# Shamir-Lab/Faucet

Measured on AMD Instinct MI355X. Metric: canonical k-mers/s (load+scan) at k=31, 100bp reads; % HBM roofline, higher is better.
Workload: dtype u64

## Files before the change

### faucet_amd/csrc/api.hip

```cpp
#include <cstdio>
#include <algorithm>
#include <string>

#include <chrono>
#include <thread>

#include "fgpu_ctx.h"

int fgpu_scan_export_impl(fgpu_ctx* ctx, void* dev_entries, uint64_t cap_entries, uint64_t* d_stamps, uint64_t* n_entries);
int fgpu_scan_import_impl(fgpu_ctx* ctx, const void* dev_entries, uint64_t n);
int fgpu_scan_download_impl(fgpu_ctx* ctx, uint64_t* keys_host, fgpu_junction* recs_host, uint64_t cap, uint64_t* n_out);

static thread_local std::string g_create_error;

int g_fgpu_trace = getenv("FGPU_TRACE") && getenv("FGPU_TRACE")[0] == '1';

int fgpu_ensure(fgpu_ctx* ctx, DevBuf* b, uint64_t bytes) {
    if (b->bytes >= bytes && b->p) return FGPU_OK;
    if (b->p) {
        FGPU_HIP(fgpu_sync_stream(ctx, ctx->stream));
        FGPU_HIP(hipFree(b->p));
        b->p = nullptr;
        b->bytes = 0;
    } else {
// ... 568 lines not shown
    ctx->host_waits = 0;
    ctx->host_wait_ms = 0;
    ctx->wait_sites.clear();
    if (ctx->short_pf) FGPU_HIP(hipMemsetAsync(ctx->short_pf, 0, ctx->short_pf_tai / 8, ctx->stream));
    if ((rc = fgpu_long_pairs_reset(ctx))) return rc;
    ctx->have_import = false;
    ctx->journal_max_read_len = 0;
    ctx->hint_in_table = false;
    ctx->hint_gen = 0;
    ctx->hint_n = ctx->hint_max_seq = 0;
    ctx->delta_ready = false;
    ctx->delta_keys = ctx->refresh_full = ctx->refresh_delta = ctx->refresh_mismatch = 0;
    ctx->sparse_links = ctx->full_links = 0;
    ctx->dbg_stall_us = getenv("FGPU_DEBUG_WALK_STALL_US") ? std::min(100000, std::max(0, atoi(getenv("FGPU_DEBUG_WALK_STALL_US")))) : 0;
    ctx->dbg_delta_check = getenv("FGPU_DEBUG_DELTA_CHECK") != nullptr;
    ctx->no_sparse_link = getenv("FGPU_NO_SPARSE_LINK") != nullptr;
    const uint64_t start_span = std::max<uint64_t>(1ULL << 18, ctx->settled_span / 4);
    ctx->window_span = ctx->prm.walk_window_span ? std::min<uint64_t>(std::max<uint64_t>(ctx->prm.walk_window_span, 64), ctx->max_span)
                                                 : std::min<uint64_t>(start_span, ctx->max_span);
    ctx->calib_left = 16;
    ctx->calib_f = ctx->calib_p = 0;
    ctx->adapt_followers = 0;
    ctx->adapt_pieces = 0;
    ctx->adapt_overflows = 0;
    ctx->adapt_vote = 0;
    ctx->calib_ovf = 0;
    ctx->span_ceiling = ~0ULL;
    ctx->repeats_seen_before = false;
    ctx->walked_pieces = 0;
    ctx->scan_batch_index = 0;
// ... 109 lines not shown
        int rc = pull_counters(ctx);
        if (rc) return rc;
        BatchBufs* const cur = ctx->cur;
        ctx->journal_max_read_len = std::max<uint64_t>(ctx->journal_max_read_len, ctx->counters_host->max_read_len);
        if (ctx->lazy_failed && (rc = scan_replay(ctx))) return rc;
        ctx->cur = cur;
        ctx->journal_on = false;
        ctx->eager_scan = true;
        journal_recycle(ctx);
        return FGPU_OK;
    }
    JournalBatch* j;
    if (!ctx->journal_pool.empty()) { j = ctx->journal_pool.back(); ctx->journal_pool.pop_back(); }
    else j = new JournalBatch();
    int rc;
    if ((rc = fgpu_ensure_b(ctx, &j->codes, cb)) || (rc = fgpu_ensure_b(ctx, &j->bad, bbytes)) || (ob && (rc = fgpu_ensure_b(ctx, &j->offs, ob)))) {
        ctx->journal_pool.push_back(j);
        return rc;
    }
    if (b->T) {
        FGPU_HIP(hipMemcpyAsync(j->codes.p, b->codes.p, cb, hipMemcpyDeviceToDevice, ctx->stream));
        FGPU_HIP(hipMemcpyAsync(j->bad.p, b->bad.p, bbytes, hipMemcpyDeviceToDevice, ctx->stream));
        if (ob) FGPU_HIP(hipMemcpyAsync(j->offs.p, b->d_offs, ob, hipMemcpyDeviceToDevice, ctx->stream));
    }
    j->T = b->T; j->n_words = b->n_words; j->n_reads = b->n_reads; j->seq = b->seq;
    ctx->journal.push_back(j);
    ctx->journal_bytes += cb + bbytes + ob;
    (void)reads;
    return FGPU_OK;
}

static int scan_replay_once(fgpu_ctx* ctx);
static int scan_replay(fgpu_ctx* ctx) {
    for (int attempt = 0;; attempt++) {
        const bool for_room = ctx->capacity_failed;
        ctx->capacity_failed = false;
        if (for_room) {
            int rc = sync_all(ctx);
// ... 12 lines not shown
}

static int scan_replay_once(fgpu_ctx* ctx) {
    ctx->in_replay = true;
    ctx->journal_on = false;
    ctx->eager_scan = true;
    ctx->lazy_failed = false;
    int rc = sync_all(ctx);
    for (BatchBufs* b : ctx->prepared) ctx->pool.push_back(b);
    ctx->prepared.clear();
    for (BatchBufs* b : ctx->to_harvest) b->stops_pending = false;
    ctx->to_harvest.clear();
    stop_queue_recycle(ctx);
    if (!rc) rc = fgpu_scan_reset(ctx);
    if (rc) { ctx->in_replay = false; return rc; }
    {
        unsigned long long ln[3] = {0, 0, 0};
        if (hipMemcpy(ln, ctx->counters->late_n, sizeof(ln), hipMemcpyDeviceToHost) == hipSuccess)
            for (int i = 0; i < 3; i++) ctx->late_acc[i] += ln[i];
    }
    FGPU_HIP(hipMemsetAsync(ctx->counters, 0, sizeof(DevCounters), ctx->stream));
    FGPU_HIP(hipMemcpyAsync(&ctx->counters->max_read_len, &ctx->journal_max_read_len, 8, hipMemcpyHostToDevice, ctx->stream));
    FGPU_HIP(fgpu_sync_stream(ctx, ctx->stream));
    const uint64_t reads_processed = ctx->scan_stats.reads_processed;
    memset(&ctx->scan_stats, 0, sizeof(ctx->scan_stats));
    ctx->scan_stats.reads_processed = reads_processed;
    memset(ctx->counters_host, 0, sizeof(DevCounters));
    ctx->scan_windows = 0;
    ctx->scan_pieces_seen = 0;
    ctx->scan_piece_base = 0;
// ... 28 lines not shown
        if (b->stops_pending && (rc = fgpu_scan_harvest(ctx, b))) {
            ctx->pool.push_back(b);
            break;
        }
        if (b->walk_pending) {
            FGPU_HIP(fgpu_sync_event(ctx, b->walk_done));
            b->walk_pending = false;
        }
        b->seq = j->seq;
        ctx->cur = b;
        b->T = j->T; b->n_words = j->n_words; b->n_reads = j->n_reads;
        b->d_offs = (const uint64_t*)j->offs.p;
        if (b->T) {
            const uint64_t cb = 2 * (b->n_words + FGPU_PADW) * 8, bbytes = (b->n_words + FGPU_PADW) * 8;
            if ((rc = fgpu_ensure_b(ctx, &b->codes, cb)) || (rc = fgpu_ensure_b(ctx, &b->bad, bbytes))) break;
            FGPU_HIP(hipMemcpyAsync(b->codes.p, j->codes.p, cb, hipMemcpyDeviceToDevice, ctx->stream));
            FGPU_HIP(hipMemcpyAsync(b->bad.p, j->bad.p, bbytes, hipMemcpyDeviceToDevice, ctx->stream));
        }
        uint64_t n_pieces = 0;
        rc = fgpu_stage_scan_pure(ctx, &n_pieces);
        if (!rc) rc = check_errors(ctx);
        if (!rc && b->pure_done) FGPU_HIP(hipEventRecord(b->pure_done, ctx->stream));
        if (!rc) rc = fgpu_scan_reserve(ctx, ctx->counters_host->n_junctions + ctx->scan_imported);
        if (!rc) {
            adapt_window(ctx);
            rc = fgpu_stage_scan_walk(ctx, b->n_pieces);
            ctx->walked_pieces += b->n_pieces;
            if (!rc) note_walked(ctx, b);
        }
        ctx->pool.push_back(b);
    }
    ctx->cur = &ctx->bb_default;
// ... 206 lines not shown
    if (dbg_host) {
        fprintf(stderr, "[host] scan: wait for the buffers' last walk %.2f ms, pack issue %.2f, pure stage issue (first half) %.2f, wait for the piece count %.2f, "
                        "pure stage issue (second half) %.2f, walk issue %.2f\n", ctx->host_ms[0], ctx->host_ms[1], ctx->host_ms[2], ctx->host_ms[3], ctx->host_ms[4], ctx->host_ms[5]);
        for (double& v : ctx->host_ms) v = 0;
    }
    int rc = pull_counters(ctx);
    if (!rc && ctx->lazy_failed) {
        rc = scan_replay(ctx);
        if (!rc) rc = pull_counters(ctx);
    }
    while (!rc && !ctx->to_harvest.empty()) rc = fgpu_scan_harvest(ctx, ctx->to_harvest.front());
    if (!rc) rc = fgpu_long_pairs_close(ctx);
    ctx->phase = 0;
    ctx->journal_on = false;
    if (!rc && !ctx->prm.walk_window_span && ctx->scan_windows > 8) ctx->settled_span = ctx->window_span;
    if (rc) return rc;
    const DevCounters& c = *ctx->counters_host;
    fgpu_scan_stats& s = ctx->scan_stats;
    s.unambiguous_reads = c.segments + ctx->carried.unambiguous_reads;
    s.reads_no_errors = c.pieces + ctx->carried.reads_no_errors;
    s.nb_jcheck_kmer = c.nb_jcheck + ctx->carried.nb_jcheck_kmer;
    s.nb_no_juncs = c.nb_no_juncs + ctx->carried.nb_no_juncs;
    s.nb_processed = c.nb_processed + ctx->carried.nb_processed;
    s.nb_skipped = c.nb_skipped + ctx->carried.nb_skipped;
    s.n_junctions = c.n_junctions + ctx->scan_imported;
    s.kmers = c.kmers + ctx->carried.kmers;
    s.reads_processed += ctx->carried.reads_processed;
    s.walk_windows = ctx->scan_windows;
    s.walk_followers = c.followers;
    s.walk_max_cluster = c.max_cluster;
// ... 285 lines not shown
```

### faucet_amd/csrc/fgpu_ctx.h

```cpp
#pragma once
#include <chrono>
#include <hip/hip_runtime.h>
#include <stdint.h>
#include <stdio.h>
#include <string.h>

#include <string>
#include <thread>
#include <vector>

#include "../../include/faucet_gpu.h"
#include <deque>

#include "fgpu_device.h"

#define FGPU_PADW 8
#define FGPU_USUAL_SPAN (1ULL << 26)
#define FGPU_MAX_SPAN (1ULL << 26)

struct DevBuf {
    void*    p = nullptr;
    uint64_t bytes = 0;
};

// ... 32 lines not shown

struct ResidentBatch {
    DevBuf codes, bad, sure;
    DevBuf fail;
    uint64_t T = 0, n_words = 0;
    uint32_t tb = 0;
};

struct DeltaList {
    DevBuf list, count;
};
#define FGPU_DELTA_RING 4

struct JournalBatch {
    DevBuf codes, bad, offs;
    uint64_t T = 0, n_words = 0, n_reads = 0, seq = 0;
};
#define FGPU_INTERNAL_REPLAY 1000

struct StopBatch {
    uint64_t seq = 0;
    fgpu_stop* data = nullptr;
    size_t n = 0, cap = 0;
};

struct LongPairs {
    int mode = 0;
    uint64_t tai = 0;
    int n_hash = 0;
    uint32_t* bits = nullptr;
// ... 158 lines not shown
    uint64_t scan_piece_base = 0;
    uint64_t scan_imported = 0;
    bool hint_in_table = false;
    uint32_t hint_gen = 0;
    uint64_t hint_n = 0, hint_max_seq = 0;
    uint64_t hint_digest[2] = {0, 0};
    DevBuf delta_filter;
    uint64_t delta_filter_bits = 0;
    bool delta_ready = false;
    uint64_t delta_keys = 0;
    uint64_t refresh_full = 0, refresh_delta = 0, refresh_mismatch = 0;
    DevBuf cand_filter;
    uint64_t sparse_links = 0, full_links = 0;
    int dbg_stall_us = 0;
    bool dbg_delta_check = false;
    bool no_sparse_link = false;
    DevBuf import_probe;
    uint64_t scan_grown = 0;

    DevCounters* counters = nullptr;
    DevCounters* counters_host = nullptr;

    fgpu_load_stats load_stats;
    uint64_t load_mark_hits = 0, load_mark_pending = 0;
    fgpu_scan_stats scan_stats;
    uint64_t scan_windows = 0;
    uint64_t scan_pieces_seen = 0;

    uint64_t adapt_followers = 0, adapt_pieces = 0;
    double host_ms[8] = {0, 0, 0, 0, 0, 0, 0, 0};
// ... 2 lines not shown
    uint64_t span_ceiling = ~0ULL;
    int adapt_vote = 0;
    uint64_t proven_span = 0;
    uint64_t adapt_overflows = 0;
    int calib_left = 0;
    uint64_t calib_f = 0, calib_p = 0;
    unsigned long long* fb_host = nullptr;
    fgpu_scan_stats carried = {};

    BatchBufs bb_default;
    BatchBufs* cur = &bb_default;
    std::vector<BatchBufs*> prepared;
    std::vector<BatchBufs*> pool;
    std::vector<BatchBufs*> all_batches;
    std::vector<JournalBatch*> journal, journal_pool;
    uint64_t journal_bytes = 0, journal_budget = 0;
    bool journal_on = false;
    bool eager_scan = false;
    bool lazy_failed = false;
    bool in_replay = false;
    bool capacity_failed = false;
    uint64_t capacity_replays = 0;
    uint32_t* short_pf = nullptr;
    uint64_t short_pf_tai = 0;
    int short_pf_hashes = 0;
    bool short_pf_lists_to_host = true;
    LongPairs lp;
    uint64_t stops_delivered = 0;
    uint64_t lp_applied_seq = 0;
    uint64_t scan_replays = 0;
// ... 155 lines not shown
```

### faucet_amd/csrc/load.hip

```cpp
#include <algorithm>

#include "fgpu_ctx.h"
#include "fgpu_flags.h"

namespace {

__device__ __forceinline__ void wave_add(unsigned long long* dst, unsigned long long v) {
    for (int o = 32; o > 0; o >>= 1) v += __shfl_down(v, o, 64);
    if (fd_lane() == 0 && v) atomicAdd(dst, v);
}

__device__ __forceinline__ void block_add(unsigned long long* dst, unsigned long long v) {
    __shared__ unsigned long long part[4];
    for (int o = 32; o > 0; o >>= 1) v += __shfl_down(v, o, 64);
    if (fd_lane() == 0) part[threadIdx.x >> 6] = v;
    __syncthreads();
    if (threadIdx.x == 0) {
        const unsigned long long t = part[0] + part[1] + part[2] + part[3];
        if (t) atomicAdd(dst, t);
    }
    __syncthreads();
}

#ifdef FGPU_FIRST_MASK_LOG2
// ... 561 lines not shown
    if (ctx->resident_bytes + cb + 2 * pb + (ctx->shard_planes ? MISS_PLANES * pb : 0) > ctx->resident_budget) {
        ctx->resident_open = false;
        return FGPU_OK;
    }
    if (ctx->resident_count == ctx->resident.size()) ctx->resident.push_back(new ResidentBatch());
    ResidentBatch& r = *ctx->resident[ctx->resident_count];
    const uint64_t fb = ctx->shard_planes ? MISS_PLANES * pb : 0;
    if (fgpu_ensure_b(ctx, &r.codes, cb) || fgpu_ensure_b(ctx, &r.bad, pb) || fgpu_ensure_b(ctx, &r.sure, pb) || (fb && fgpu_ensure_b(ctx, &r.fail, fb))) {
        (void)hipGetLastError();
        ctx->resident_open = false;
        return FGPU_OK;
    }
    r.T = bb.T;
    r.n_words = bb.n_words;
    r.tb = ctx->cur_tb;
    FGPU_HIP(hipMemcpyAsync(r.codes.p, bb.codes.p, cb, hipMemcpyDeviceToDevice, ctx->stream));
    FGPU_HIP(hipMemcpyAsync(r.bad.p, bb.bad.p, pb, hipMemcpyDeviceToDevice, ctx->stream));
    FGPU_HIP(hipMemcpyAsync(r.sure.p, bb.sure.p, pb, hipMemcpyDeviceToDevice, ctx->stream));
    if (fb) FGPU_HIP(hipMemcpyAsync(r.fail.p, bb.fail.p, fb, hipMemcpyDeviceToDevice, ctx->stream));
    ctx->resident_count++;
    ctx->resident_bytes += cb + 2 * pb + fb;
    return FGPU_OK;
}

int fgpu_load_sweep(fgpu_ctx* ctx) {
    if (ctx->epoch_positions == 0) return FGPU_OK;
    if (ctx->rec_layout) FGPU_LAUNCH("carry_update", k_carry_from_rec, 8192, 256, ctx->rec, ctx->prm.tai / 32);
    else FGPU_LAUNCH("carry_update", k_carry_from_first, 4096, 256, ctx->pair, (const uint4*)ctx->first, ctx->prm.tai);
    ctx->swept_positions += ctx->epoch_positions;
    ctx->epoch_positions = 0;
    return FGPU_OK;
}

int fgpu_stage_load(fgpu_ctx* ctx) {
// ... 133 lines not shown
```

### faucet_amd/csrc/scan_pure.hip

```cpp
#include <algorithm>

#include "fgpu_ctx.h"
#include "fgpu_flags.h"

namespace {

__device__ __forceinline__ void wave_add(unsigned long long* dst, unsigned long long v) {
    for (int o = 32; o > 0; o >>= 1) v += __shfl_down(v, o, 64);
    if (fd_lane() == 0 && v) atomicAdd(dst, v);
}

__device__ __forceinline__ void block_add(unsigned long long* dst, unsigned long long v) {
    __shared__ unsigned long long part[4];
    for (int o = 32; o > 0; o >>= 1) v += __shfl_down(v, o, 64);
    if (fd_lane() == 0) part[threadIdx.x >> 6] = v;
    __syncthreads();
    if (threadIdx.x == 0) {
        const unsigned long long t = part[0] + part[1] + part[2] + part[3];
        if (t) atomicAdd(dst, t);
    }
    __syncthreads();
}

__global__ void __launch_bounds__(256) k_scan_same(const uint64_t* __restrict__ codes, const uint64_t* __restrict__ kept_codes, uint64_t n_code_words,
                                                   const uint64_t* __restrict__ bad, const uint64_t* __restrict__ kept_bad, uint64_t n_words,
                                                   uint32_t* same) {
    bool differ = false;
    for (uint64_t i = (uint64_t)blockIdx.x * blockDim.x + threadIdx.x; i < n_code_words; i += (uint64_t)gridDim.x * blockDim.x) {
        differ |= codes[i] != kept_codes[i];
        if (i < n_words) differ |= bad[i] != kept_bad[i];
    }
    if (__ballot(differ) && fd_lane() == 0) *same = 0;
}

__global__ void __launch_bounds__(256) k_scan_valid(const uint64_t* __restrict__ codes, const uint64_t* __restrict__ bad,
                                                    uint64_t T, uint64_t n_words, FdParams fp, const uint32_t* __restrict__ bloom,
                                                    const uint64_t* __restrict__ sure, const uint32_t* __restrict__ same,
                                                    uint64_t* __restrict__ valid, DevCounters* cnt) {
    unsigned long long n_ok = 0, n_reused = 0;
    const uint64_t total = n_words * 64;
    const bool reuse = sure && *same != 0;
    for (uint64_t p = (uint64_t)blockIdx.x * blockDim.x + threadIdx.x; p < total; p += (uint64_t)gridDim.x * blockDim.x) {
        bool ok = p < T && fd_window_ok(bad, p, fp.k);
        bool v = false;
        if (ok) {
            n_ok++;
            if (reuse && ((sure[p >> 6] >> (p & 63)) & 1ULL)) {
// ... 427 lines not shown

}

void fgpu_touch_scan_pure() {
    hipFuncAttributes attr;
    (void)hipFuncGetAttributes(&attr, (const void*)k_scan_same);
}

int fgpu_util_probe_stage3(fgpu_ctx* ctx, const uint64_t* d_kmers, uint64_t n, int mode, signed char* d_out) {
    FGPU_LAUNCH("probe_stage3", k_probe_stage3, fgpu_blocks(n, 256), 256, d_kmers, n, mode, ctx->fd, (const uint32_t*)ctx->bloo2, d_out);
    return FGPU_OK;
}

int fgpu_stage_scan_pure(fgpu_ctx* ctx, uint64_t* n_pieces) {
    BatchBufs& bb = *ctx->cur;
    *n_pieces = 0;
    bb.n_pieces = 0;
    if (bb.T == 0) return FGPU_OK;
    const uint64_t wb = (bb.n_words + FGPU_PADW) * 8;
    int rc;
    DevBuf* planes[] = {&bb.valid, &bb.pm, &bb.ps, &bb.ff, &bb.fb, &bb.cf0, &bb.cf1, &bb.cb0, &bb.cb1, &bb.inF, &bb.inB, &bb.lk, &bb.nF, &bb.nB, &bb.need};
    for (DevBuf* b : planes)
        if ((rc = fgpu_ensure_b(ctx, b, wb))) return rc;
    if ((rc = fgpu_ensure_b(ctx, &bb.ps_prefix, (bb.n_words + FGPU_PADW + bb.n_words / SCAN_BLOCK + 2) * 4))) return rc;
    const double t_a = fgpu_host_now();
    FGPU_HIP(hipMemsetAsync(bb.valid.p, 0, wb, ctx->stream));
    FGPU_HIP(hipMemsetAsync(bb.pm.p, 0, wb, ctx->stream));
    FGPU_HIP(hipMemsetAsync(bb.ps.p, 0, wb, ctx->stream));

    const unsigned grid = fgpu_grid(bb.n_words * 64, 256);
    const unsigned wgrid = fgpu_grid(bb.n_words, 256);
    if ((rc = fgpu_util_count_segments(ctx, ctx->fd.k + 2 * ctx->fd.j + 1))) return rc;
    const ResidentBatch* kept = ctx->scan_batch_index < ctx->resident_count ? ctx->resident[ctx->scan_batch_index] : nullptr;
    ctx->scan_batch_index++;
    if (kept && (kept->T != bb.T || kept->n_words != bb.n_words)) kept = nullptr;
    if (kept) {
        if ((rc = fgpu_ensure_b(ctx, &bb.same, 64))) return rc;
        FGPU_HIP(hipMemsetAsync(bb.same.p, 0x01, 4, ctx->stream));
        const uint64_t ncw = 2 * bb.n_words;
        FGPU_LAUNCH("scan_same", k_scan_same, fgpu_grid(ncw, 256), 256, (const uint64_t*)bb.codes.p, (const uint64_t*)kept->codes.p, ncw,
                    (const uint64_t*)bb.bad.p, (const uint64_t*)kept->bad.p, bb.n_words, (uint32_t*)bb.same.p);
    }
    FGPU_LAUNCH("scan_valid", k_scan_valid, grid, 256, (const uint64_t*)bb.codes.p, (const uint64_t*)bb.bad.p, bb.T, bb.n_words, ctx->fd,
                (const uint32_t*)ctx->bloo2, kept ? (const uint64_t*)kept->sure.p : (const uint64_t*)nullptr,
                kept ? (const uint32_t*)bb.same.p : (const uint32_t*)nullptr, (uint64_t*)bb.valid.p, ctx->counters);
    const int check_segment = ctx->fd.k < 2 * ctx->fd.j + 2;
    FGPU_LAUNCH("scan_pieces", k_scan_pieces, wgrid, 256, (const uint64_t*)bb.valid.p, (const uint64_t*)bb.bad.p, bb.n_words, ctx->fd,
                check_segment, (unsigned long long*)bb.pm.p, (uint64_t*)bb.ps.p, ctx->counters);
    uint32_t* prefix = (uint32_t*)bb.ps_prefix.p;
    uint32_t* block_sums = prefix + bb.n_words + FGPU_PADW;
    const uint32_t nblk = fgpu_blocks(bb.n_words + 1, SCAN_BLOCK);
    const uint64_t nw1 = bb.n_words + 1;
    FGPU_LAUNCH("prefix_block", k_prefix_block, nblk, SCAN_BLOCK, (const uint64_t*)bb.ps.p, nw1, prefix, block_sums);
    FGPU_LAUNCH("prefix_sums", k_prefix_sums, 1, SCAN_BLOCK, block_sums, nblk);
    FGPU_LAUNCH("prefix_apply", k_prefix_apply, fgpu_blocks(nw1, 256), 256, prefix, (const uint32_t*)block_sums, nw1);
    FGPU_HIP(hipMemcpyAsync(ctx->counters_host, ctx->counters, sizeof(DevCounters), hipMemcpyDeviceToHost, ctx->stream));
// ... 48 lines not shown
```

### faucet_amd/csrc/scan_walk.hip

```cpp
#include <cstring>
#include <algorithm>

#include "fgpu_ctx.h"
#include "fgpu_flags.h"

#include <rocprim/rocprim.hpp>

namespace {

constexpr uint64_t J_EMPTY = ~0ULL;
constexpr uint64_t J_KEYMASK = (1ULL << 62) - 1;
constexpr uint32_t U_INF = 0xFFFFFFFFu;
constexpr uint64_t J_PROBE_LIMIT = 1ULL << 14;
constexpr int STAMP_SHIFT = 20;
constexpr uint64_t STAMP_FAKE = (1ULL << STAMP_SHIFT) - 1;

struct JTable {
    uint64_t* keys;
    uint8_t* recs;
    uint64_t* stamps;
    uint64_t mask;
    uint32_t* filter;
    uint64_t filter_mask;
};
// ... 83 lines not shown
    }
    return false;
}

__device__ __forceinline__ uint32_t uf_find(uint32_t* parent, uint32_t x) {
    uint32_t p = ld_agent(&parent[x]);
    while (p != x) {
        uint32_t gp = ld_agent(&parent[p]);
        if (gp != p) atomicMin(&parent[x], gp);
        x = p;
        p = gp;
    }
    return x;
}

__device__ __forceinline__ void uf_union(uint32_t* parent, uint32_t a, uint32_t b) {
    for (;;) {
        a = uf_find(parent, a);
        b = uf_find(parent, b);
        if (a == b) return;
        if (a < b) { uint32_t t = a; a = b; b = t; }
        uint32_t old = atomicCAS(&parent[a], a, b);
        if (old == a) return;
    }
}

constexpr int W_OWNER_BITS = 24;
constexpr uint64_t W_OWNER_MASK = (1ULL << W_OWNER_BITS) - 1;
constexpr uint64_t W_EPOCH_MASK = 0xFFULL << 56;
constexpr uint32_t W_NO_OWNER = (uint32_t)W_OWNER_MASK;
__device__ __forceinline__ uint32_t wt_filter_bit(const WTable& wt, uint32_t h32) { return (h32 * 0x85EBCA6Bu) >> wt.fshift; }

__device__ __forceinline__ void wt_register(const WTable& wt, uint32_t* parent, uint32_t h32, uint32_t piece, DevCounters* cnt) {
    const unsigned long long mine = (unsigned long long)(wt.epoch | ((uint64_t)h32 << W_OWNER_BITS) | (uint64_t)piece);
    uint64_t s = (uint64_t)h32 & wt.mask;
    for (uint64_t n = 0; n <= wt.mask; n++) {
        unsigned long long v = wt.keys[s];
        if ((v & W_EPOCH_MASK) != wt.epoch) {
// ... 62 lines not shown

struct DeltaSrc {
    const uint32_t* list[FGPU_DELTA_RING];
    const unsigned long long* count[FGPU_DELTA_RING];
};

__global__ void __launch_bounds__(256) k_walk_register(Planes pl, FdParams fp, WTable wt, uint32_t* parent, uint64_t lo, uint64_t hi,
                                                       uint64_t pos_end, DevCounters* cnt, unsigned word_blocks, unsigned piece_blocks, DeltaSrc ds) {
    const WinDesc wd = make_window(pl, lo, hi);
    if (blockIdx.x < word_blocks) {
        const uint64_t w = (wd.lo >> 6) + (uint64_t)blockIdx.x * blockDim.x + threadIdx.x;
        if (w * 64 >= pos_end) return;
        unsigned long long m = pl.pm[w] & (pl.inF[w] | pl.inB[w] | pl.ff[w] | pl.fb[w]);
        if (w == (wd.lo >> 6)) m &= ~0ULL << (wd.lo & 63);
        if ((w + 1) * 64 > pos_end) m &= (1ULL << (pos_end & 63)) - 1;
        while (m) {
            const int b = __builtin_ctzll(m);
            m &= m - 1;
            const uint64_t p = w * 64 + (uint64_t)b;
            uint32_t li;
            uint2 pc;
            if (piece_in_window(pl, wd, p, li, pc)) wt_register(wt, parent, pl.kh[p], li, cnt);
        }
    } else if (blockIdx.x < word_blocks + piece_blocks) {
        const uint32_t li = (blockIdx.x - word_blocks) * blockDim.x + threadIdx.x;
        if (li >= wd.n) return;
        const uint2 pc = pl.pieces[wd.first_piece + li];
        const uint32_t len = pc.y + (uint32_t)fp.k - 1;
        wt_register(wt, parent, pl.kh[pc.x + (len / 2 - (uint32_t)fp.k / 2)], li, cnt);
        for (uint32_t q = (uint32_t)fp.max_spacer - 1; q < pc.y; q++) wt_register(wt, parent, pl.kh[pc.x + q], li, cnt);
    } else {
        const uint64_t t = (uint64_t)(blockIdx.x - word_blocks - piece_blocks) * blockDim.x + threadIdx.x;
        const uint64_t stride = (uint64_t)(gridDim.x - word_blocks - piece_blocks) * blockDim.x;
        for (int r = 0; r < FGPU_DELTA_RING; r++) {
            if (!ds.list[r]) continue;
            const uint64_t n = *ds.count[r];
            for (uint64_t i = t; i < n; i += stride) wt_register(wt, nullptr, ds.list[r][i], W_NO_OWNER, cnt);
        }
    }
}

__global__ void __launch_bounds__(256) k_walk_link(Planes pl, FdParams fp, WTable wt, uint32_t* parent, uint64_t lo, uint64_t hi,
                                                   uint64_t pos_end, uint32_t* roots_state) {
    const WinDesc wd = make_window(pl, lo, hi);
    if (roots_state && blockIdx.x == 0 && threadIdx.x == 0) { roots_state[0] = 0; roots_state[1] = 0; }
    const uint64_t base0 = wd.lo & ~63ULL;
    constexpr int U = 4;
    for (uint64_t base = base0 + (uint64_t)blockIdx.x * (256 * U); base < pos_end; base += (uint64_t)gridDim.x * (256 * U)) {
        uint64_t p[U];
        uint32_t h[U], fw[U];
        bool act[U];
#pragma unroll
        for (int u = 0; u < U; u++) {
            p[u] = base + (uint64_t)u * 256 + threadIdx.x;
            act[u] = p[u] >= wd.lo && p[u] < pos_end && ((pl.pm[p[u] >> 6] >> (p[u] & 63)) & 1ULL);
        }
#pragma unroll
        for (int u = 0; u < U; u++) h[u] = act[u] ? pl.kh[p[u]] : 0u;
#pragma unroll
        for (int u = 0; u < U; u++) {
            const uint32_t b = wt_filter_bit(wt, h[u]);
            fw[u] = act[u] ? ((wt.bits[b >> 5] >> (b & 31)) & 1u) : 0u;
        }
#pragma unroll
        for (int u = 0; u < U; u++) {
            bool hit = false;
            if (fw[u]) {
                uint64_t slot = 0;
                uint32_t owner = wt_owner(wt, h[u], slot);
                if (owner != U_INF) {
                    uint32_t li;
                    uint2 pc;
                    if (piece_in_window(pl, wd, p[u], li, pc)) {
                        hit = true;
                        if (owner == W_NO_OWNER) {
                            const unsigned long long mine = (unsigned long long)(wt.epoch | ((uint64_t)h[u] << W_OWNER_BITS) | (uint64_t)li);
                            owner = (uint32_t)(atomicMin((unsigned long long*)&wt.keys[slot], mine) & W_OWNER_MASK);
                        }
                        if (owner != li && owner != W_NO_OWNER) uf_union(parent, li, owner);
                    }
                }
            }
            const uint64_t m = __ballot(hit);
            if (fd_lane() == 0 && p[u] < ((pos_end + 63) & ~63ULL)) pl.lk[p[u] >> 6] = m;
        }
    }
}

constexpr int CAND_FILTER_LOG2 = 27;
__device__ __forceinline__ uint32_t cand_bit(uint32_t h32) { return (h32 * 0xC2B2AE35u) >> (32 - CAND_FILTER_LOG2); }

__global__ void __launch_bounds__(256) k_cand_mark(const uint64_t* __restrict__ pm, const uint64_t* __restrict__ inF, const uint64_t* __restrict__ inB,
                                                   const uint64_t* __restrict__ ff, const uint64_t* __restrict__ fb, const uint32_t* __restrict__ kh,
                                                   uint64_t n_words, const uint2* __restrict__ pieces, uint64_t n_pieces, FdParams fp,
                                                   uint32_t* __restrict__ filt, unsigned word_blocks) {
    if (blockIdx.x < word_blocks) {
        for (uint64_t w = (uint64_t)blockIdx.x * blockDim.x + threadIdx.x; w < n_words; w += (uint64_t)word_blocks * blockDim.x) {
            unsigned long long m = pm[w] & (inF[w] | inB[w] | ff[w] | fb[w]);
            while (m) {
// ... 55 lines not shown
            if (!piece_in_window(pl, wd, p, li, pc)) continue;
            out |= 1ULL << b;
            if (owner == W_NO_OWNER) {
                const unsigned long long mine = (unsigned long long)(wt.epoch | ((uint64_t)h << W_OWNER_BITS) | (uint64_t)li);
                owner = (uint32_t)(atomicMin((unsigned long long*)&wt.keys[slot], mine) & W_OWNER_MASK);
            }
            if (owner != li && owner != W_NO_OWNER) uf_union(parent, li, owner);
        }
        lk_out[w] = out;
    }
}

__global__ void __launch_bounds__(256) k_walk_cluster(const uint32_t* __restrict__ parent, uint32_t* count, uint32_t* head,
                                                      uint32_t* __restrict__ flat, uint32_t* __restrict__ next, Planes pl, uint64_t lo,
                                                      uint64_t hi, WinDesc* wd_out, DevCounters* cnt, uint32_t* weight, uint32_t heavy_w,
                                                      uint32_t* __restrict__ root_list, uint32_t* roots_state) {
    const WinDesc wd = make_window(pl, lo, hi);
    const uint32_t n = wd.n;
    if (blockIdx.x == 0 && threadIdx.x == 0) {
        *wd_out = wd;
        cnt->pad2 = 0;
    }
    for (uint32_t i = blockIdx.x * blockDim.x + threadIdx.x; i < n; i += gridDim.x * blockDim.x) {
        uint32_t r = i;
        for (;;) { uint32_t pr = parent[r]; if (pr == r) break; r = pr; }
        flat[i] = r;
        if (r != i) {
            next[i] = atomicExch(&head[r], i);
            atomicAdd(&count[r], 1u);
        }
        {
            const bool is_root = r == i;
            const unsigned long long m = __ballot(is_root);
            if (m) {
                const int first = __builtin_ctzll(m);
// ... 1800 lines not shown
            const unsigned total = s_wave[0] + s_wave[1] + s_wave[2] + s_wave[3];
            s_base = total ? atomicAdd(count, (unsigned long long)total) : 0ULL;
        }
        __syncthreads();
        unsigned long long at = s_base + (incl - mine);
        for (int q = 0; q < wave; q++) at += s_wave[q];
        while (m) {
            const int b = __builtin_ctzll(m);
            m &= m - 1;
            list[at++] = kh[w * 64 + (uint64_t)b];
        }
        __syncthreads();
    }
}

__global__ void __launch_bounds__(256) k_walk_reset_uf(uint32_t* parent, uint32_t* count, uint32_t* head, uint32_t* par_fail, uint32_t n, uint4* wbits,
                                                       uint32_t wbits_vec) {
    for (uint32_t a = blockIdx.x * blockDim.x + threadIdx.x; a < n; a += gridDim.x * blockDim.x) {
        parent[a] = a;
        count[a] = 0;
        head[a] = U_INF;
        par_fail[a] = 0;
    }
    for (uint32_t a = blockIdx.x * blockDim.x + threadIdx.x; a < wbits_vec; a += gridDim.x * blockDim.x) wbits[a] = make_uint4(0, 0, 0, 0);
}

__global__ void __launch_bounds__(256) k_fill_u64(uint64_t* p, uint64_t n, uint64_t v) {
    uint64_t i = (uint64_t)blockIdx.x * blockDim.x + threadIdx.x;
    uint64_t stride = (uint64_t)gridDim.x * blockDim.x;
    for (; i < n; i += stride) p[i] = v;
}
__global__ void __launch_bounds__(256) k_iota_u32(uint32_t* p, uint64_t n) {
// ... 657 lines not shown
                    }
                if (lo) {
                    ds.list[FGPU_DELTA_RING - 1] = (const uint32_t*)mine_list.list.p;
                    ds.count[FGPU_DELTA_RING - 1] = (const unsigned long long*)mine_list.count.p;
                }
            }
            const unsigned word_blocks = fgpu_blocks((pos_end - (lo & ~63ULL) + 63) / 64, 256);
            const unsigned piece_blocks = fgpu_blocks(max_pieces, 256);
            static const unsigned delta_per_block = getenv("FGPU_DELTA_PER_BLOCK") ? (unsigned)std::max(1, atoi(getenv("FGPU_DELTA_PER_BLOCK"))) : 1024u;
            const unsigned delta_blocks = refresh_window ? 64u : (unsigned)std::min<uint64_t>(4096, std::max<uint64_t>(64, delta_est / delta_per_block));
            FGPU_LAUNCH("walk_lookup", k_walk_register, word_blocks + piece_blocks + delta_blocks, 256, pl, ctx->fd, wt, uf_parent, lo, hi, pos_end, ctx->counters,
                        word_blocks, piece_blocks, ds);
        }
        uint32_t* const roots_state = ctx->cl_roots;
        uint32_t* const root_list = ctx->cl_roots + 16;
        if (cand_ok && lo == 0) {
            const uint64_t link_words = ((pos_end + 63) >> 6) - (lo >> 6);
            FGPU_LAUNCH("walk_link", k_walk_link_sparse, std::min(fgpu_blocks(link_words, 256), 4096u), 256, pl, ctx->fd, wt, uf_parent, lo, hi, pos_end, roots_state,
                        (const uint64_t*)bb.cand.p, (uint64_t*)bb.lk.p);
            ctx->sparse_links++;
            if (ctx->dbg_delta_check) {
                uint64_t* copy = nullptr;
                unsigned long long* out = nullptr;
                FGPU_HIP(hipMalloc(&copy, link_words * 8));
                FGPU_HIP(hipMalloc(&out, 32));
                FGPU_HIP(hipMemsetAsync(out, 0, 32, walk_stream));
                FGPU_HIP(hipMemcpyAsync(copy, (const uint64_t*)bb.lk.p + (lo >> 6), link_words * 8, hipMemcpyDeviceToDevice, walk_stream));
                hipLaunchKernelGGL(k_walk_link, dim3(std::min(fgpu_blocks(pos_end - (lo & ~63ULL), 1024), 4096u)), dim3(256), 0, walk_stream, pl, ctx->fd, wt, uf_parent, lo, hi, pos_end,
                                   (uint32_t*)nullptr);
                hipLaunchKernelGGL(k_dbg_diff, dim3(64), dim3(256), 0, walk_stream, (const uint64_t*)copy, (const uint64_t*)bb.lk.p + (lo >> 6), link_words, out, 0);
                unsigned long long h[4] = {0, 0, 0, 0};
                FGPU_HIP(hipMemcpyAsync(h, out, 32, hipMemcpyDeviceToHost, walk_stream));
                FGPU_HIP(hipStreamSynchronize(walk_stream));
                ctx->refresh_mismatch += h[0];
                if (h[0]) fprintf(stderr, "[fgpu] sparse link pass: %llu lk words differ from the full pass's, batch %llu window at %llu\n", h[0], (unsigned long long)bb.seq, (unsigned long long)lo);
                (void)hipFree(copy); (void)hipFree(out);
            }
        } else {
            FGPU_LAUNCH("walk_link", k_walk_link, std::min(fgpu_blocks(pos_end - (lo & ~63ULL), 1024), 4096u), 256, pl, ctx->fd, wt, uf_parent, lo, hi, pos_end, roots_state);
            if (ctx->refresh_snapshot) ctx->full_links++;
        }
        const uint32_t ko_heavy = (dbg_walk || !ctx->walk_ko || !(ctx->walk_ko_always || ctx->counters_host->max_cluster >= ctx->walk_ko)) ? 0u : ctx->walk_ko;
        static const int ko_avg_env = getenv("FGPU_WALK_KO_AVG") ? std::min(255, std::max(0, atoi(getenv("FGPU_WALK_KO_AVG")))) : -1;
        static const int ko_avg_min_env = getenv("FGPU_WALK_KO_AVG_MIN") ? std::min(255, std::max(1, atoi(getenv("FGPU_WALK_KO_AVG_MIN")))) : -1;
        const bool repeats_seen = ctx->counters_host->walk_parallel * 50 > ctx->counters_host->walked_pieces ||
                                  (ctx->walk_ko_always && ctx->counters_host->walked_pieces < (1ULL << 17) && ctx->delta_next >= 2 && ctx->repeats_seen_before);
        if (repeats_seen) ctx->repeats_seen_before = true;
        const uint32_t ko_total = std::min<uint32_t>(ctx->walk_ko_weight, 0xFFFFu);
        const uint32_t ko_avg = ko_avg_env >= 0 ? (uint32_t)ko_avg_env : repeats_seen ? 8u : 12u;
        const uint32_t ko_total_rep = ko_avg_min_env > 0 ? (uint32_t)ko_avg_min_env : repeats_seen ? 16u : std::min<uint32_t>(255u, 3 * ko_total / 8);
        const uint32_t ko_heavy_w = (ko_heavy && ko_total) ? (ko_total | (ko_avg << 16) | (ko_total_rep << 24)) : 0u;
        FGPU_LAUNCH("walk_cluster", k_walk_cluster, cluster_grid, 256, (const uint32_t*)uf_parent, cl_count, cl_offset, ctx->cl_fill,
                    ctx->cl_members, pl, lo, hi, (WinDesc*)ctx->wdesc, ctx->counters, cl_fail, ko_heavy_w, root_list, roots_state);
        static const uint32_t ko_ticket = getenv("FGPU_KO_TICKET") ? (uint32_t)std::max(64, atoi(getenv("FGPU_KO_TICKET")) / 64 * 64) : 64u;
        const uint32_t heavy = (dbg_walk || ko_heavy) ? 0u : ctx->walk_heavy;
        KoTables kt;
        kt.hk_key = ctx->ko_hk;
        kt.hk_head = ctx->ko_hk + ctx->ko_hk_cap;
        kt.hk_turn = ctx->ko_hk + 2 * (size_t)ctx->ko_hk_cap;
        kt.hk_mask = ctx->ko_hk_cap - 1;
        kt.occ_id = (uint64_t*)ctx->ko_occ;
        kt.occ_entry = (uint32_t*)(kt.occ_id + ctx->ko_occ_cap);
        kt.occ_rank = kt.occ_entry + ctx->ko_occ_cap;
        kt.occ_next = kt.occ_rank + ctx->ko_occ_cap;
        kt.occ_cap = ctx->ko_occ_cap;
        kt.trace = nullptr;
#ifdef FGPU_KO_TRACE
        if (!ctx->ko_trace.p) {
// ... 126 lines not shown
            FGPU_LAUNCH("walk_ko", k_walk_ko, ko_grid, 64, pl, ctx->fd, jt, (const uint32_t*)ctx->cl_fill, (const uint32_t*)cl_count, (const WinDesc*)ctx->wdesc,
                        seq_base, (const uint32_t*)ctx->bloo2, ctx->counters, kt, ko_heavy, ko_ticket, (const uint32_t*)cl_fail, ko_heavy_w,
                        (const uint32_t*)ot.state, (const uint32_t*)ot.longp, ovw_rounds);
        if (heavy)
            FGPU_LAUNCH("walk_commit", k_walk_par<WALK_COMMIT>, walk_grid_w, 64, pl, ctx->fd, jt, (const uint32_t*)ctx->cl_fill, (const uint32_t*)cl_count, cl_fail,
                        (const WinDesc*)ctx->wdesc, (const uint32_t*)ctx->bloo2, ctx->counters, heavy);
        {
            const uint64_t w_first = lo >> 6, w_last = std::min<uint64_t>(bb.n_words, (pos_end + 63) / 64);
            FGPU_LAUNCH("walk_delta", k_delta_collect, (unsigned)std::min<uint64_t>(fgpu_blocks(w_last - w_first, 256), 256), 256, (unsigned long long*)bb.cr.p,
                        (const uint32_t*)bb.kh.p, w_first, w_last, (uint32_t*)mine_list.list.p, (unsigned long long*)mine_list.count.p, pl,
                        (const WinDesc*)ctx->wdesc, ctx->counters, (uint32_t)ctx->scan_windows);
        }
        FGPU_HIP(hipEventRecord(ctx->ev_walked, walk_stream));
        FGPU_HIP(hipStreamWaitEvent(ctx->cstream, ctx->ev_walked, 0));
        ctx->launch_stream = ctx->cstream;
        FGPU_LAUNCH("walk_clean", k_walk_reset_uf, std::min(256u, fgpu_blocks(max_pieces, 256)), 256, uf_parent, cl_count, cl_offset, cl_fail, (uint32_t)max_pieces, (uint4*)wt.bits, (uint32_t)((1u << ctx->wbits_log2) / 128));
        ctx->launch_stream = walk_stream;
        FGPU_HIP(hipEventRecord(ctx->ev_uf_reset[parity], ctx->cstream));
        if (serial_clean) FGPU_HIP(hipStreamWaitEvent(walk_stream, ctx->ev_uf_reset[parity], 0));
        ctx->scan_windows++;
        if (ctx->calib_left > 0 && !ctx->prm.walk_window_span) {
            FGPU_HIP(hipMemcpyAsync(ctx->fb_host, &ctx->counters->followers, 8, hipMemcpyDeviceToHost, walk_stream));
            FGPU_HIP(hipMemcpyAsync(ctx->fb_host + 1, &ctx->counters->walked_pieces, 8, hipMemcpyDeviceToHost, walk_stream));
            FGPU_HIP(hipMemcpyAsync(ctx->fb_host + 2, &ctx->counters->ko_overflows, 8, hipMemcpyDeviceToHost, walk_stream));
            FGPU_HIP(fgpu_sync_stream(ctx, walk_stream));
            const uint64_t f = ctx->fb_host[0] - ctx->calib_f, p = ctx->fb_host[1] - ctx->calib_p;
            if (ctx->fb_host[2] > ctx->calib_ovf && span_now > 4096) {
                ctx->calib_ovf = ctx->fb_host[2];
                ctx->calib_f = ctx->fb_host[0];
                ctx->calib_p = ctx->fb_host[1];
                span_now = std::max<uint64_t>(4096, span_now / 4);
// ... 363 lines not shown
```

Measured before the change: 5.832 billion.

## Skip redundant journal/resident copies, skip re-linking registered positions, shrink UF reset

Resident batches now take ownership of the batch buffers through a pointer swap instead of device-to-device copies. Journal entries copy codes and bad bits only when the batch differs from the kept resident batch, and otherwise point replay at the resident buffers. The link kernel skips positions already registered in the word-table pass, using the lk plane it wrote. The union-find reset now clears only the number of pieces actually in the window rather than max_pieces. An optional debug path cross-checks the skipping link pass against a full pass. Risks include buffer aliasing from the swap, replay depending on the resident buffers staying valid, and extra host syncs during replay.

```diff
diff --git a/faucet_amd/csrc/api.hip b/faucet_amd/csrc/api.hip
--- a/faucet_amd/csrc/api.hip
+++ b/faucet_amd/csrc/api.hip
@@ -606,6 +606,8 @@
     ctx->sparse_links = ctx->full_links = 0;
     ctx->dbg_stall_us = getenv("FGPU_DEBUG_WALK_STALL_US") ? std::min(100000, std::max(0, atoi(getenv("FGPU_DEBUG_WALK_STALL_US")))) : 0;
     ctx->dbg_delta_check = getenv("FGPU_DEBUG_DELTA_CHECK") != nullptr;
+    ctx->dbg_link_check = getenv("FGPU_DEBUG_LINK_CHECK") != nullptr;
+    ctx->link_skipped = ctx->link_probed = 0;
     ctx->no_sparse_link = getenv("FGPU_NO_SPARSE_LINK") != nullptr;
     const uint64_t start_span = std::max<uint64_t>(1ULL << 18, ctx->settled_span / 4);
     ctx->window_span = ctx->prm.walk_window_span ? std::min<uint64_t>(std::max<uint64_t>(ctx->prm.walk_window_span, 64), ctx->max_span)
@@ -745,14 +747,15 @@
     if (!ctx->journal_pool.empty()) { j = ctx->journal_pool.back(); ctx->journal_pool.pop_back(); }
     else j = new JournalBatch();
     int rc;
-    if ((rc = fgpu_ensure_b(ctx, &j->codes, cb)) || (rc = fgpu_ensure_b(ctx, &j->bad, bbytes)) || (ob && (rc = fgpu_ensure_b(ctx, &j->offs, ob)))) {
+    if ((rc = fgpu_ensure_b(ctx, &j->codes, cb)) || (rc = fgpu_ensure_b(ctx, &j->bad, bbytes)) || (ob && (rc = fgpu_ensure_b(ctx, &j->offs, ob))) ||
+        (rc = fgpu_ensure(ctx, &j->same, 64))) {
         ctx->journal_pool.push_back(j);
         return rc;
     }
+    j->kept = -1;
     if (b->T) {
-        FGPU_HIP(hipMemcpyAsync(j->codes.p, b->codes.p, cb, hipMemcpyDeviceToDevice, ctx->stream));
-        FGPU_HIP(hipMemcpyAsync(j->bad.p, b->bad.p, bbytes, hipMemcpyDeviceToDevice, ctx->stream));
         if (ob) FGPU_HIP(hipMemcpyAsync(j->offs.p, b->d_offs, ob, hipMemcpyDeviceToDevice, ctx->stream));
+        ctx->journal_cur = j;
     }
     j->T = b->T; j->n_words = b->n_words; j->n_reads = b->n_reads; j->seq = b->seq;
     ctx->journal.push_back(j);
@@ -795,6 +798,16 @@
     stop_queue_recycle(ctx);
     if (!rc) rc = fgpu_scan_reset(ctx);
     if (rc) { ctx->in_replay = false; return rc; }
+    std::vector<const ResidentBatch*> src(ctx->journal.size(), nullptr);
+    for (size_t i = 0; i < ctx->journal.size(); i++) {
+        const JournalBatch* j = ctx->journal[i];
+        if (j->kept < 0) continue;
+        uint32_t same = 0;
+        FGPU_HIP(hipMemcpy(&same, j->same.p, 4, hipMemcpyDeviceToHost));
+        if (!same) continue;
+        if ((uint64_t)j->kept >= ctx->resident.size()) { ctx->in_replay = false; ctx->err = "journal entry refers to a missing kept batch"; return FGPU_ERR_STATE; }
+        src[i] = ctx->resident[j->kept];
+    }
     {
         unsigned long long ln[3] = {0, 0, 0};
         if (hipMemcpy(ln, ctx->counters->late_n, sizeof(ln), hipMemcpyDeviceToHost) == hipSuccess)
@@ -853,8 +866,8 @@
         if (b->T) {
             const uint64_t cb = 2 * (b->n_words + FGPU_PADW) * 8, bbytes = (b->n_words + FGPU_PADW) * 8;
             if ((rc = fgpu_ensure_b(ctx, &b->codes, cb)) || (rc = fgpu_ensure_b(ctx, &b->bad, bbytes))) break;
-            FGPU_HIP(hipMemcpyAsync(b->codes.p, j->codes.p, cb, hipMemcpyDeviceToDevice, ctx->stream));
-            FGPU_HIP(hipMemcpyAsync(b->bad.p, j->bad.p, bbytes, hipMemcpyDeviceToDevice, ctx->stream));
+            FGPU_HIP(hipMemcpyAsync(b->codes.p, src[i] ? src[i]->codes.p : j->codes.p, cb, hipMemcpyDeviceToDevice, ctx->stream));
+            FGPU_HIP(hipMemcpyAsync(b->bad.p, src[i] ? src[i]->bad.p : j->bad.p, bbytes, hipMemcpyDeviceToDevice, ctx->stream));
         }
         uint64_t n_pieces = 0;
         rc = fgpu_stage_scan_pure(ctx, &n_pieces);
@@ -1091,6 +1104,9 @@
     ctx->phase = 0;
     ctx->journal_on = false;
     if (!rc && !ctx->prm.walk_window_span && ctx->scan_windows > 8) ctx->settled_span = ctx->window_span;
+    if (!rc && ctx->dbg_link_check)
+        fprintf(stderr, "[fgpu] link check: %llu registered positions skipped, %llu probed, %llu mismatches in all\n", (unsigned long long)ctx->link_skipped,
+                (unsigned long long)ctx->link_probed, (unsigned long long)ctx->refresh_mismatch);
     if (rc) return rc;
     const DevCounters& c = *ctx->counters_host;
     fgpu_scan_stats& s = ctx->scan_stats;
diff --git a/faucet_amd/csrc/fgpu_ctx.h b/faucet_amd/csrc/fgpu_ctx.h
--- a/faucet_amd/csrc/fgpu_ctx.h
+++ b/faucet_amd/csrc/fgpu_ctx.h
@@ -70,6 +70,8 @@
 
 struct JournalBatch {
     DevBuf codes, bad, offs;
+    DevBuf same;
+    int64_t kept = -1;
     uint64_t T = 0, n_words = 0, n_reads = 0, seq = 0;
 };
 #define FGPU_INTERNAL_REPLAY 1000
@@ -258,6 +260,8 @@
     uint64_t sparse_links = 0, full_links = 0;
     int dbg_stall_us = 0;
     bool dbg_delta_check = false;
+    bool dbg_link_check = false;
+    uint64_t link_skipped = 0, link_probed = 0;
     bool no_sparse_link = false;
     DevBuf import_probe;
     uint64_t scan_grown = 0;
@@ -290,6 +294,7 @@
     std::vector<BatchBufs*> pool;
     std::vector<BatchBufs*> all_batches;
     std::vector<JournalBatch*> journal, journal_pool;
+    JournalBatch* journal_cur = nullptr;
     uint64_t journal_bytes = 0, journal_budget = 0;
     bool journal_on = false;
     bool eager_scan = false;
diff --git a/faucet_amd/csrc/load.hip b/faucet_amd/csrc/load.hip
--- a/faucet_amd/csrc/load.hip
+++ b/faucet_amd/csrc/load.hip
@@ -599,10 +599,10 @@
     r.T = bb.T;
     r.n_words = bb.n_words;
     r.tb = ctx->cur_tb;
-    FGPU_HIP(hipMemcpyAsync(r.codes.p, bb.codes.p, cb, hipMemcpyDeviceToDevice, ctx->stream));
-    FGPU_HIP(hipMemcpyAsync(r.bad.p, bb.bad.p, pb, hipMemcpyDeviceToDevice, ctx->stream));
-    FGPU_HIP(hipMemcpyAsync(r.sure.p, bb.sure.p, pb, hipMemcpyDeviceToDevice, ctx->stream));
-    if (fb) FGPU_HIP(hipMemcpyAsync(r.fail.p, bb.fail.p, fb, hipMemcpyDeviceToDevice, ctx->stream));
+    std::swap(r.codes, bb.codes);
+    std::swap(r.bad, bb.bad);
+    std::swap(r.sure, bb.sure);
+    if (fb) std::swap(r.fail, bb.fail);
     ctx->resident_count++;
     ctx->resident_bytes += cb + 2 * pb + fb;
     return FGPU_OK;
diff --git a/faucet_amd/csrc/scan_pure.hip b/faucet_amd/csrc/scan_pure.hip
--- a/faucet_amd/csrc/scan_pure.hip
+++ b/faucet_amd/csrc/scan_pure.hip
@@ -31,6 +31,18 @@
         if (i < n_words) differ |= bad[i] != kept_bad[i];
     }
     if (__ballot(differ) && fd_lane() == 0) *same = 0;
+}
+
+__global__ void __launch_bounds__(256) k_journal_copy(const uint32_t* __restrict__ same, uint32_t* __restrict__ j_same, const uint64_t* __restrict__ codes,
+                                                      uint64_t* __restrict__ j_codes, uint64_t n_code_words, const uint64_t* __restrict__ bad,
+                                                      uint64_t* __restrict__ j_bad, uint64_t n_words) {
+    const uint32_t s = *same;
+    if (blockIdx.x == 0 && threadIdx.x == 0) *j_same = s;
+    if (s) return;
+    for (uint64_t i = (uint64_t)blockIdx.x * blockDim.x + threadIdx.x; i < n_code_words; i += (uint64_t)gridDim.x * blockDim.x) {
+        j_codes[i] = codes[i];
+        if (i < n_words) j_bad[i] = bad[i];
+    }
 }
 
 __global__ void __launch_bounds__(256) k_scan_valid(const uint64_t* __restrict__ codes, const uint64_t* __restrict__ bad,
@@ -488,6 +500,8 @@
 
 int fgpu_stage_scan_pure(fgpu_ctx* ctx, uint64_t* n_pieces) {
     BatchBufs& bb = *ctx->cur;
+    JournalBatch* const jb = ctx->journal_cur;
+    ctx->journal_cur = nullptr;
     *n_pieces = 0;
     bb.n_pieces = 0;
     if (bb.T == 0) return FGPU_OK;
@@ -508,12 +522,21 @@
     const ResidentBatch* kept = ctx->scan_batch_index < ctx->resident_count ? ctx->resident[ctx->scan_batch_index] : nullptr;
     ctx->scan_batch_index++;
     if (kept && (kept->T != bb.T || kept->n_words != bb.n_words)) kept = nullptr;
+    const uint64_t cb = 2 * (bb.n_words + FGPU_PADW) * 8;
     if (kept) {
         if ((rc = fgpu_ensure_b(ctx, &bb.same, 64))) return rc;
         FGPU_HIP(hipMemsetAsync(bb.same.p, 0x01, 4, ctx->stream));
         const uint64_t ncw = 2 * bb.n_words;
         FGPU_LAUNCH("scan_same", k_scan_same, fgpu_grid(ncw, 256), 256, (const uint64_t*)bb.codes.p, (const uint64_t*)kept->codes.p, ncw,
                     (const uint64_t*)bb.bad.p, (const uint64_t*)kept->bad.p, bb.n_words, (uint32_t*)bb.same.p);
+        if (jb) {
+            jb->kept = (int64_t)(ctx->scan_batch_index - 1);
+            FGPU_LAUNCH("journal_copy", k_journal_copy, std::min(1024u, fgpu_grid(cb / 8, 256)), 256, (const uint32_t*)bb.same.p, (uint32_t*)jb->same.p,
+                        (const uint64_t*)bb.codes.p, (uint64_t*)jb->codes.p, cb / 8, (const uint64_t*)bb.bad.p, (uint64_t*)jb->bad.p, cb / 16);
+        }
+    } else if (jb) {
+        FGPU_HIP(hipMemcpyAsync(jb->codes.p, bb.codes.p, cb, hipMemcpyDeviceToDevice, ctx->stream));
+        FGPU_HIP(hipMemcpyAsync(jb->bad.p, bb.bad.p, cb / 2, hipMemcpyDeviceToDevice, ctx->stream));
     }
     FGPU_LAUNCH("scan_valid", k_scan_valid, grid, 256, (const uint64_t*)bb.codes.p, (const uint64_t*)bb.bad.p, bb.T, bb.n_words, ctx->fd,
                 (const uint32_t*)ctx->bloo2, kept ? (const uint64_t*)kept->sure.p : (const uint64_t*)nullptr,
diff --git a/faucet_amd/csrc/scan_walk.hip b/faucet_amd/csrc/scan_walk.hip
--- a/faucet_amd/csrc/scan_walk.hip
+++ b/faucet_amd/csrc/scan_walk.hip
@@ -121,14 +121,14 @@
     return x;
 }
 
-__device__ __forceinline__ void uf_union(uint32_t* parent, uint32_t a, uint32_t b) {
+__device__ __forceinline__ bool uf_union(uint32_t* parent, uint32_t a, uint32_t b) {
     for (;;) {
         a = uf_find(parent, a);
         b = uf_find(parent, b);
-        if (a == b) return;
+        if (a == b) return false;
         if (a < b) { uint32_t t = a; a = b; b = t; }
         uint32_t old = atomicCAS(&parent[a], a, b);
-        if (old == a) return;
+        if (old == a) return true;
     }
 }
 
@@ -221,14 +221,19 @@
         unsigned long long m = pl.pm[w] & (pl.inF[w] | pl.inB[w] | pl.ff[w] | pl.fb[w]);
         if (w == (wd.lo >> 6)) m &= ~0ULL << (wd.lo & 63);
         if ((w + 1) * 64 > pos_end) m &= (1ULL << (pos_end & 63)) - 1;
+        unsigned long long reg = 0;
         while (m) {
             const int b = __builtin_ctzll(m);
             m &= m - 1;
             const uint64_t p = w * 64 + (uint64_t)b;
             uint32_t li;
             uint2 pc;
-            if (piece_in_window(pl, wd, p, li, pc)) wt_register(wt, parent, pl.kh[p], li, cnt);
-        }
+            if (piece_in_window(pl, wd, p, li, pc)) {
+                wt_register(wt, parent, pl.kh[p], li, cnt);
+                reg |= 1ULL << b;
+            }
+        }
+        pl.lk[w] = reg;
     } else if (blockIdx.x < word_blocks + piece_blocks) {
         const uint32_t li = (blockIdx.x - word_blocks) * blockDim.x + threadIdx.x;
         if (li >= wd.n) return;
@@ -247,8 +252,9 @@
     }
 }
 
+template <bool SKIP>
 __global__ void __launch_bounds__(256) k_walk_link(Planes pl, FdParams fp, WTable wt, uint32_t* parent, uint64_t lo, uint64_t hi,
-                                                   uint64_t pos_end, uint32_t* roots_state) {
+                                                   uint64_t pos_end, uint32_t* roots_state, uint64_t* lk_out, unsigned long long* dbg) {
     const WinDesc wd = make_window(pl, lo, hi);
     if (roots_state && blockIdx.x == 0 && threadIdx.x == 0) { roots_state[0] = 0; roots_state[1] = 0; }
     const uint64_t base0 = wd.lo & ~63ULL;
@@ -256,11 +262,14 @@
     for (uint64_t base = base0 + (uint64_t)blockIdx.x * (256 * U); base < pos_end; base += (uint64_t)gridDim.x * (256 * U)) {
         uint64_t p[U];
         uint32_t h[U], fw[U];
-        bool act[U];
+        bool act[U], reg[U];
 #pragma unroll
         for (int u = 0; u < U; u++) {
             p[u] = base + (uint64_t)u * 256 + threadIdx.x;
-            act[u] = p[u] >= wd.lo && p[u] < pos_end && ((pl.pm[p[u] >> 6] >> (p[u] & 63)) & 1ULL);
+            const bool in = p[u] >= wd.lo && p[u] < pos_end;
+            const uint64_t pmw = in ? pl.pm[p[u] >> 6] : 0ULL, lkw = (SKIP && in) ? pl.lk[p[u] >> 6] : 0ULL;
+            reg[u] = (lkw >> (p[u] & 63)) & 1ULL;
+            act[u] = ((pmw >> (p[u] & 63)) & 1ULL) && !reg[u];
         }
 #pragma unroll
         for (int u = 0; u < U; u++) h[u] = act[u] ? pl.kh[p[u]] : 0u;
@@ -271,7 +280,7 @@
         }
 #pragma unroll
         for (int u = 0; u < U; u++) {
-            bool hit = false;
+            bool hit = reg[u];
             if (fw[u]) {
                 uint64_t slot = 0;
                 uint32_t owner = wt_owner(wt, h[u], slot);
@@ -284,12 +293,16 @@
                             const unsigned long long mine = (unsigned long long)(wt.epoch | ((uint64_t)h[u] << W_OWNER_BITS) | (uint64_t)li);
                             owner = (uint32_t)(atomicMin((unsigned long long*)&wt.keys[slot], mine) & W_OWNER_MASK);
                         }
-                        if (owner != li && owner != W_NO_OWNER) uf_union(parent, li, owner);
+                        if (owner != li && owner != W_NO_OWNER && uf_union(parent, li, owner) && !SKIP && dbg) atomicAdd(&dbg[2], 1ULL);
                     }
                 }
             }
             const uint64_t m = __ballot(hit);
-            if (fd_lane() == 0 && p[u] < ((pos_end + 63) & ~63ULL)) pl.lk[p[u] >> 6] = m;
+            if (fd_lane() == 0 && p[u] < ((pos_end + 63) & ~63ULL)) lk_out[p[u] >> 6] = m;
+            if (SKIP && dbg) {
+                const uint64_t rm = __ballot(reg[u]), am = __ballot(act[u]);
+                if (fd_lane() == 0 && (rm | am)) { atomicAdd(&dbg[0], (unsigned long long)__popcll(rm)); atomicAdd(&dbg[1], (unsigned long long)__popcll(am)); }
+            }
         }
     }
 }
@@ -375,11 +388,12 @@
 __global__ void __launch_bounds__(256) k_walk_cluster(const uint32_t* __restrict__ parent, uint32_t* count, uint32_t* head,
                                                       uint32_t* __restrict__ flat, uint32_t* __restrict__ next, Planes pl, uint64_t lo,
                                                       uint64_t hi, WinDesc* wd_out, DevCounters* cnt, uint32_t* weight, uint32_t heavy_w,
-                                                      uint32_t* __restrict__ root_list, uint32_t* roots_state) {
+                                                      uint32_t* __restrict__ root_list, uint32_t* roots_state, uint32_t* uf_n) {
     const WinDesc wd = make_window(pl, lo, hi);
     const uint32_t n = wd.n;
     if (blockIdx.x == 0 && threadIdx.x == 0) {
         *wd_out = wd;
+        *uf_n = n;
         cnt->pad2 = 0;
     }
     for (uint32_t i = blockIdx.x * blockDim.x + threadIdx.x; i < n; i += gridDim.x * blockDim.x) {
@@ -2210,8 +2224,9 @@
     }
 }
 
-__global__ void __launch_bounds__(256) k_walk_reset_uf(uint32_t* parent, uint32_t* count, uint32_t* head, uint32_t* par_fail, uint32_t n, uint4* wbits,
-                                                       uint32_t wbits_vec) {
+__global__ void __launch_bounds__(256) k_walk_reset_uf(uint32_t* parent, uint32_t* count, uint32_t* head, uint32_t* par_fail, const uint32_t* uf_n,
+                                                       uint32_t cap, uint4* wbits, uint32_t wbits_vec) {
+    const uint32_t n = min(*uf_n, cap);
     for (uint32_t a = blockIdx.x * blockDim.x + threadIdx.x; a < n; a += gridDim.x * blockDim.x) {
         parent[a] = a;
         count[a] = 0;
@@ -2899,6 +2914,7 @@
         }
         uint32_t* const roots_state = ctx->cl_roots;
         uint32_t* const root_list = ctx->cl_roots + 16;
+        uint32_t* const uf_n = ctx->cl_roots + 2 + parity;
         if (cand_ok && lo == 0) {
             const uint64_t link_words = ((pos_end + 63) >> 6) - (lo >> 6);
             FGPU_LAUNCH("walk_link", k_walk_link_sparse, std::min(fgpu_blocks(link_words, 256), 4096u), 256, pl, ctx->fd, wt, uf_parent, lo, hi, pos_end, roots_state,
@@ -2911,8 +2927,8 @@
                 FGPU_HIP(hipMalloc(&out, 32));
                 FGPU_HIP(hipMemsetAsync(out, 0, 32, walk_stream));
                 FGPU_HIP(hipMemcpyAsync(copy, (const uint64_t*)bb.lk.p + (lo >> 6), link_words * 8, hipMemcpyDeviceToDevice, walk_stream));
-                hipLaunchKernelGGL(k_walk_link, dim3(std::min(fgpu_blocks(pos_end - (lo & ~63ULL), 1024), 4096u)), dim3(256), 0, walk_stream, pl, ctx->fd, wt, uf_parent, lo, hi, pos_end,
-                                   (uint32_t*)nullptr);
+                hipLaunchKernelGGL(k_walk_link<false>, dim3(std::min(fgpu_blocks(pos_end - (lo & ~63ULL), 1024), 4096u)), dim3(256), 0, walk_stream, pl, ctx->fd, wt, uf_parent, lo, hi,
+                                   pos_end, (uint32_t*)nullptr, (uint64_t*)bb.lk.p, (unsigned long long*)nullptr);
                 hipLaunchKernelGGL(k_dbg_diff, dim3(64), dim3(256), 0, walk_stream, (const uint64_t*)copy, (const uint64_t*)bb.lk.p + (lo >> 6), link_words, out, 0);
                 unsigned long long h[4] = {0, 0, 0, 0};
                 FGPU_HIP(hipMemcpyAsync(h, out, 32, hipMemcpyDeviceToHost, walk_stream));
@@ -2922,8 +2938,30 @@
                 (void)hipFree(copy); (void)hipFree(out);
             }
         } else {
-            FGPU_LAUNCH("walk_link", k_walk_link, std::min(fgpu_blocks(pos_end - (lo & ~63ULL), 1024), 4096u), 256, pl, ctx->fd, wt, uf_parent, lo, hi, pos_end, roots_state);
+            const unsigned link_grid = std::min(fgpu_blocks(pos_end - (lo & ~63ULL), 1024), 4096u);
+            unsigned long long* dbg = nullptr;
+            if (ctx->dbg_link_check) {
+                FGPU_HIP(hipMalloc(&dbg, 32));
+                FGPU_HIP(hipMemsetAsync(dbg, 0, 32, walk_stream));
+            }
+            FGPU_LAUNCH("walk_link", k_walk_link<true>, link_grid, 256, pl, ctx->fd, wt, uf_parent, lo, hi, pos_end, roots_state, (uint64_t*)bb.lk.p, dbg);
             if (ctx->refresh_snapshot) ctx->full_links++;
+            if (dbg) {
+                const uint64_t w0 = lo >> 6, w1 = (pos_end + 63) >> 6;
+                uint64_t* full = nullptr;
+                FGPU_HIP(hipMalloc(&full, w1 * 8));
+                hipLaunchKernelGGL(k_walk_link<false>, dim3(link_grid), dim3(256), 0, walk_stream, pl, ctx->fd, wt, uf_parent, lo, hi, pos_end, (uint32_t*)nullptr, full, dbg);
+                hipLaunchKernelGGL(k_dbg_diff, dim3(64), dim3(256), 0, walk_stream, (const uint64_t*)full + w0, (const uint64_t*)bb.lk.p + w0, w1 - w0, dbg, 3);
+                unsigned long long h[4] = {0, 0, 0, 0};
+                FGPU_HIP(hipMemcpyAsync(h, dbg, 32, hipMemcpyDeviceToHost, walk_stream));
+                FGPU_HIP(hipStreamSynchronize(walk_stream));
+                ctx->link_skipped += h[0];
+                ctx->link_probed += h[1];
+                ctx->refresh_mismatch += h[2] + h[3];
+                if (h[2] + h[3]) fprintf(stderr, "[fgpu] link pass: %llu unions of the full pass merged sets, %llu lk words differ, batch %llu window at %llu\n", h[2], h[3],
+                                         (unsigned long long)bb.seq, (unsigned long long)lo);
+                (void)hipFree(full); (void)hipFree(dbg);
+            }
         }
         const uint32_t ko_heavy = (dbg_walk || !ctx->walk_ko || !(ctx->walk_ko_always || ctx->counters_host->max_cluster >= ctx->walk_ko)) ? 0u : ctx->walk_ko;
         static const int ko_avg_env = getenv("FGPU_WALK_KO_AVG") ? std::min(255, std::max(0, atoi(getenv("FGPU_WALK_KO_AVG")))) : -1;
@@ -2936,7 +2974,7 @@
         const uint32_t ko_total_rep = ko_avg_min_env > 0 ? (uint32_t)ko_avg_min_env : repeats_seen ? 16u : std::min<uint32_t>(255u, 3 * ko_total / 8);
         const uint32_t ko_heavy_w = (ko_heavy && ko_total) ? (ko_total | (ko_avg << 16) | (ko_total_rep << 24)) : 0u;
         FGPU_LAUNCH("walk_cluster", k_walk_cluster, cluster_grid, 256, (const uint32_t*)uf_parent, cl_count, cl_offset, ctx->cl_fill,
-                    ctx->cl_members, pl, lo, hi, (WinDesc*)ctx->wdesc, ctx->counters, cl_fail, ko_heavy_w, root_list, roots_state);
+                    ctx->cl_members, pl, lo, hi, (WinDesc*)ctx->wdesc, ctx->counters, cl_fail, ko_heavy_w, root_list, roots_state, uf_n);
         static const uint32_t ko_ticket = getenv("FGPU_KO_TICKET") ? (uint32_t)std::max(64, atoi(getenv("FGPU_KO_TICKET")) / 64 * 64) : 64u;
         const uint32_t heavy = (dbg_walk || ko_heavy) ? 0u : ctx->walk_heavy;
         KoTables kt;
@@ -3093,7 +3131,7 @@
         FGPU_HIP(hipEventRecord(ctx->ev_walked, walk_stream));
         FGPU_HIP(hipStreamWaitEvent(ctx->cstream, ctx->ev_walked, 0));
         ctx->launch_stream = ctx->cstream;
-        FGPU_LAUNCH("walk_clean", k_walk_reset_uf, std::min(256u, fgpu_blocks(max_pieces, 256)), 256, uf_parent, cl_count, cl_offset, cl_fail, (uint32_t)max_pieces, (uint4*)wt.bits, (uint32_t)((1u << ctx->wbits_log2) / 128));
+        FGPU_LAUNCH("walk_clean", k_walk_reset_uf, std::min(256u, fgpu_blocks(max_pieces, 256)), 256, uf_parent, cl_count, cl_offset, cl_fail, (const uint32_t*)uf_n, (uint32_t)max_pieces, (uint4*)wt.bits, (uint32_t)((1u << ctx->wbits_log2) / 128));
         ctx->launch_stream = walk_stream;
         FGPU_HIP(hipEventRecord(ctx->ev_uf_reset[parity], ctx->cstream));
         if (serial_clean) FGPU_HIP(hipStreamWaitEvent(walk_stream, ctx->ev_uf_reset[parity], 0));
```

New measurement: 5.890 billion (median of 6 runs). Within noise of the previous version (+1.0%).
